# Mehooz/vision4leg

Measured on AMD Instinct MI355X. Metric: PPO env-steps/s (encoder+update, sim excluded), higher is better.
Workload: dtype f16; 1 GPU; ppo_locotransformer thin-goal: LocoTransformer S=93 A=6, E=32 envs x T=512, B=1024, 3 opt epochs; net=loco, envs_per_gpu=32, horizon=512, minibatch=1024, opt_epochs=3, parallelism=dp1, includes_rollout_inference=True, logp_old=recorded at action time (target_pf forward skipped; SURVEY 8d declared saving)

## Files before the change

vision4leg_amd/csrc/bwd.h:

```cpp
#pragma once
#include "infer.h"

namespace v4l {

struct BwdLayer {
  const void *w2t, *w1t, *wot, *wint;
  const float *g1, *g2;
  const float* dy;
  const float *s_qkv, *s_P, *s_xh1, *s_rs1, *s_xh2, *s_rs2;
  const void* s_f;
  void *o_dz2, *o_df, *o_dz1, *o_dqkv;
  float* o_dx;
  float *gp2, *bp2, *gp1, *bp1;
};

struct BwdLayerStack { BwdLayer l[2]; };

struct BwdHead {
  const void *w2t, *w1t, *w0t;
  const float* dout;
  const float *s_h1, *s_h0;
  float *o_dh1, *o_dh0;
};
struct BwdTail {
// ... 632 lines not shown
  LAY_STAMP(8);
  }
  if constexpr (TAIL) {
    __syncthreads();
    {
      f32x4 acc[MT][1];
      zero_acc(acc);
      block_gemm<T, MT, 1, 2>(acc, at, LY::LDX, (const T*)tl.wupt, 64, nt1, lane, ring_up);
      const int n4 = wave * 16 + qr;
#pragma unroll
      for (int mt = 0; mt < MT; ++mt) {
        const int row = mt * 16 + fr;
        const int sm = row / NTOK, t = row - sm * NTOK;
        const bool ok = row < nrows && t > 0;
        const int64_t o = ok ? ((int64_t)(s0 + sm) * 16 + (t - 1)) * TD + n4 : 0;
        const float4 m = tm_c3[mt];
        if (ok)
          st4(tl.o_dc3 + o, m.x > 0.f ? acc[mt][0][0] : 0.f, m.y > 0.f ? acc[mt][0][1] : 0.f, m.z > 0.f ? acc[mt][0][2] : 0.f,
              m.w > 0.f ? acc[mt][0][3] : 0.f);
      }
    }
    float* dt = big;
    T* dh = reinterpret_cast<T*>(big + 16 * LY::LDX);
    GemmRing<T, 4, 8> ring_f2 = gemm_prefetch<T, 4, 8>((const T*)tl.wf2t, 256, nt4, lane);
    __syncthreads();
#pragma unroll
    for (int k = 0; k < 4; ++k) {
      const int idx = tid + k * 256, r = idx >> 6, c = idx & 63;
      dt[r * LY::LDX + c] = r < ns && tm_x0[k] > 0.f ? at[(r * NTOK) * LY::LDX + c] : 0.f;
    }
    __syncthreads();
    f32x4 acc[1][4];
    auto masked = [&](const float4 (&m)[4], T* dst, float* save) {
      const bool ok = fr < ns;
#pragma unroll
      for (int j = 0; j < 4; ++j) {
        const int n4 = nt4[j] * 16 + qr;
        const float d0 = m[j].x > 0.f ? acc[0][j][0] : 0.f, d1 = m[j].y > 0.f ? acc[0][j][1] : 0.f;
        const float d2 = m[j].z > 0.f ? acc[0][j][2] : 0.f, d3 = m[j].w > 0.f ? acc[0][j][3] : 0.f;
        if (dst != nullptr) st4(dst + fr * LY::LDF + n4, d0, d1, d2, d3);
        if (ok) st4(save + (int64_t)(s0 + fr) * 256 + n4, d0, d1, d2, d3);
      }
    };
    zero_acc(acc);
    block_gemm<T, 1, 4, 2>(acc, dt, LY::LDX, (const T*)tl.wpt, 64, nt4, lane, ring_pr);
    masked(tm_e1, dh, tl.o_dhc);
    __syncthreads();
    zero_acc(acc);
    block_gemm<T, 1, 4, 8>(acc, dh, LY::LDF, (const T*)tl.wf2t, 256, nt4, lane, ring_f2);
    masked(tm_e0, (T*)nullptr, tl.o_de0);
  }
  LAY_STAMP(9);
}


struct BwdConv {
  const void* w3d;
  const void* w2d[4];
  const void* image;
  const int* rowidx;
  const float *c1, *c2;
  const float* dc3;
  float *slab1, *slab2, *slab3;
  float *bslab1, *bslab2, *bslab3;
  int n;
  void *t_dc2, *t_dc1;
};
template <typename T> struct BwdConvLds {
  static constexpr bool B16 = sizeof(T) == 2;
  static constexpr int LF = 64 + 4;
  static constexpr int LC1 = 32 + (B16 ? 8 : 0);
  static constexpr int IMGP = B16 ? 1 : 2;
  static constexpr int LT = 64 + (B16 ? 8 : 4);
  static constexpr int LP2 = 64 + (B16 ? 8 : 4);
  static constexpr int LP1 = 256 + (B16 ? 8 : 4);
  static constexpr size_t dc3_b = (size_t)17 * LT * sizeof(T);
  static constexpr size_t c2_b = (size_t)36 * LF * 4;
  static constexpr size_t dc2_b = (size_t)48 * LT * sizeof(T);
  static constexpr size_t dc2T_b = (size_t)64 * LP2 * sizeof(T);
  static constexpr size_t c1_b = ((size_t)225 * LC1 * sizeof(T) + 15) / 16 * 16;
  static constexpr size_t dc1_b = (size_t)32 * LP1 * sizeof(T);
  static constexpr size_t img_b = (size_t)(4 / IMGP) * 4096 * sizeof(T);
  static constexpr size_t w2_b = B16 ? (size_t)4 * 32 * 256 * sizeof(T) : 0;
  static constexpr size_t bytes = dc3_b + c2_b + dc2_b + dc2T_b + c1_b + dc1_b + img_b + w2_b;
  static_assert(bytes <= 160 * 1024, "one block per CU");
};

template <typename T> __device__ __forceinline__ typename Frag<T>::type frag_of(const float (&v)[8]) {
  typename Frag<T>::type f;
  if constexpr (sizeof(T) == 2) {
#pragma unroll
    for (int j = 0; j < 8; ++j) f[j] = (T)v[j];
  } else {
#pragma unroll
    for (int j = 0; j < 8; ++j) f.v[j] = v[j];
  }
  return f;
}
template <typename H>
__device__ __forceinline__ typename Frag<H>::type frag_of_t(const H (&v)[8]) {
  static_assert(sizeof(H) == 2, "16-bit operand type");
  typename Frag<H>::type f;
#pragma unroll
  for (int j = 0; j < 8; ++j) f[j] = v[j];
  return f;
}
__device__ __forceinline__ f32x8 frag_of_t(const float (&v)[8]) { return frag_of<float>(v); }

template <typename T, int MT, int NT, int KS, int KS0 = 0, int PDEPTH = 4, class RowF>
__device__ __forceinline__ void gather_gemm(f32x4 (&acc)[MT][NT], const T* __restrict__ W, int Kp, int nt0, int lane, RowF arow) {
  typedef typename Frag<T>::type frag_t;
  constexpr int PD = NT >= 2 ? 2 : (KS < PDEPTH ? KS : PDEPTH);
  const int fr = lane & 15, fg = (lane >> 4) * 8;
  const T* wrow = W + (int64_t)(nt0 * 16 + fr) * Kp + fg + KS0 * 32;
  frag_t fb[PD][NT];
#pragma unroll
  for (int d = 0; d < PD; ++d)
#pragma unroll
    for (int j = 0; j < NT; ++j) fb[d][j] = *reinterpret_cast<const frag_t*>(wrow + (int64_t)j * 16 * Kp + d * 32);
#pragma unroll
  for (int ks = 0; ks < KS; ++ks) {
    frag_t cur[NT];
#pragma unroll
    for (int j = 0; j < NT; ++j) cur[j] = fb[ks % PD][j];
    if (ks + PD < KS) {
#pragma unroll
      for (int j = 0; j < NT; ++j) fb[ks % PD][j] = *reinterpret_cast<const frag_t*>(wrow + (int64_t)j * 16 * Kp + (ks + PD) * 32);
    }
#pragma unroll
    for (int mt = 0; mt < MT; ++mt) {
      const frag_t fa = *reinterpret_cast<const frag_t*>(arow(mt, (ks + KS0) >> 1) + ((ks + KS0) & 1) * 32 + fg);
#pragma unroll
      for (int j = 0; j < NT; ++j)
        mma_k32(acc[mt][j], cur[j], fa);
    }
  }
}

#ifdef V4L_INFER_TIMING
#define CONV_STAMP(i) do { if (blockIdx.x == 0 && threadIdx.x == 0 && smp == 3 * (int)gridDim.x) g_inf_stamps[16 + (i)] = clock64(); } while (0)
#else
#define CONV_STAMP(i)
#endif
template <typename T, bool A16 = false>
__global__ __launch_bounds__(512) void bwd_conv_kernel(BwdConv a) {
  static_assert(!A16 || sizeof(T) == 2, "A16: activations saved in the bf16 operand type");
  typedef BwdConvLds<T> LY;
  typedef typename Frag<T>::type frag_t;
  constexpr int NTH = 512;
  extern __shared__ __attribute__((aligned(16))) unsigned char smem[];
  T* sdc3 = reinterpret_cast<T*>(smem);
  float* sc2 = reinterpret_cast<float*>(smem + LY::dc3_b);
  T* sdc2t = reinterpret_cast<T*>(smem + LY::dc3_b + LY::c2_b);
  T* sdc2T = reinterpret_cast<T*>(smem + LY::dc3_b + LY::c2_b + LY::dc2_b);
  constexpr size_t o_c1 = LY::dc3_b + LY::c2_b + LY::dc2_b + LY::dc2T_b;
  T* sc1 = reinterpret_cast<T*>(smem + o_c1);
  T* sdc1T = reinterpret_cast<T*>(smem + o_c1 + LY::c1_b);
  T* simg = reinterpret_cast<T*>(smem + o_c1 + LY::c1_b + LY::dc1_b);
  T* sw2 = reinterpret_cast<T*>(smem + o_c1 + LY::c1_b + LY::dc1_b + LY::img_b);
  const int tid = threadIdx.x, lane = tid & 63, wave = tid >> 6;
  const int fr = lane & 15, g = lane >> 4, qr = g * 4;
  const int kt2 = wave * 4;
  const int ch1 = wave >> 1, th1 = wave & 1;
  f32x4 acc2[4][4], acc1[2][2];
#pragma unroll
  for (int t = 0; t < 4; ++t) {
#pragma unroll
    for (int c = 0; c < 4; ++c) acc2[t][c] = f32x4{0.f, 0.f, 0.f, 0.f};
    acc1[t >> 1][t & 1] = f32x4{0.f, 0.f, 0.f, 0.f};
  }
  float b2r[4] = {0.f, 0.f, 0.f, 0.f};
  float b1r[4] = {0.f, 0.f, 0.f, 0.f};
  for (int i = tid; i < 12 * LY::LT; i += NTH) sdc2t[36 * LY::LT + i] = (T)0.f;
  for (int i = tid; i < 64 * LY::LP2; i += NTH) sdc2T[i] = (T)0.f;
  for (int i = tid; i < 32 * LY::LP1; i += NTH) sdc1T[i] = (T)0.f;
  for (int i = tid; i < LY::LT; i += NTH) sdc3[16 * LY::LT + i] = (T)0.f;
  constexpr int CH = 4 / LY::IMGP;

  constexpr int V = 16 / sizeof(T);
  constexpr int N4 = 225 * 8, PT = (N4 + NTH - 1) / NTH;
  constexpr int N8 = 225 * 4, PT8 = (N8 + NTH - 1) / NTH;
  typedef typename Frag<T>::type chunk_t;
  float4 hv0 = float4{0.f, 0.f, 0.f, 0.f}, hv1 = hv0, cv[A16 ? 1 : PT];
  chunk_t h16 = {}, c16[A16 ? PT8 : 1] = {};
  auto load_next = [&](int sm) {
    const float* g3 = a.dc3 + (int64_t)sm * 16 * 64;
    if constexpr (A16) {
      const chunk_t* g2 = reinterpret_cast<const chunk_t*>(reinterpret_cast<const T*>(a.c2) + (int64_t)sm * 36 * 64);
      const chunk_t* g1 = reinterpret_cast<const chunk_t*>(reinterpret_cast<const T*>(a.c1) + (int64_t)sm * 225 * 32);
      h16 = g2[tid < 288 ? tid : 0];
      if (tid >= 256) hv1 = *reinterpret_cast<const float4*>(g3 + (tid - 256) * 4);
#pragma unroll
      for (int k = 0; k < PT8; ++k) {
        const int i8 = tid + k * NTH;
        c16[k] = g1[i8 < N8 ? i8 : 0];
      }
    } else {
      const float* g2 = a.c2 + (int64_t)sm * 36 * 64;
      const float* g1 = a.c1 + (int64_t)sm * 225 * 32;
      hv0 = *reinterpret_cast<const float4*>(g2 + tid * 4);
      if (tid >= 256) hv1 = *reinterpret_cast<const float4*>(g3 + (tid - 256) * 4);
      else if (tid < 64) hv1 = *reinterpret_cast<const float4*>(g2 + (512 + tid) * 4);
#pragma unroll
      for (int k = 0; k < PT; ++k) {
        const int i4 = tid + k * NTH;
        cv[k] = *reinterpret_cast<const float4*>(g1 + (i4 < N4 ? i4 : 0) * 4);
      }
    }
  };
  auto store_next = [&]() {
    if constexpr (A16) {
      if (tid < 288) {
        float* d = sc2 + (tid >> 3) * LY::LF + (tid & 7) * 8;
        *reinterpret_cast<float4*>(d) = float4{(float)h16[0], (float)h16[1], (float)h16[2], (float)h16[3]};
        *reinterpret_cast<float4*>(d + 4) = float4{(float)h16[4], (float)h16[5], (float)h16[6], (float)h16[7]};
      }
      if (tid >= 256) st4(sdc3 + ((tid - 256) >> 4) * LY::LT + (tid & 15) * 4, hv1.x, hv1.y, hv1.z, hv1.w);
#pragma unroll
      for (int k = 0; k < PT8; ++k) {
        const int i8 = tid + k * NTH;
        if (i8 < N8) *reinterpret_cast<chunk_t*>(sc1 + (i8 >> 2) * LY::LC1 + (i8 & 3) * 8) = c16[k];
      }
    } else {
      *reinterpret_cast<float4*>(sc2 + (tid >> 4) * LY::LF + (tid & 15) * 4) = hv0;
      if (tid >= 256) st4(sdc3 + ((tid - 256) >> 4) * LY::LT + (tid & 15) * 4, hv1.x, hv1.y, hv1.z, hv1.w);
      else if (tid < 64) *reinterpret_cast<float4*>(sc2 + (32 + (tid >> 4)) * LY::LF + (tid & 15) * 4) = hv1;
#pragma unroll
      for (int k = 0; k < PT; ++k) {
        const int i4 = tid + k * NTH;
        if (i4 < N4) st4(sc1 + (i4 >> 3) * LY::LC1 + (i4 & 7) * 4, cv[k].x, cv[k].y, cv[k].z, cv[k].w);
      }
    }
  };
  {
    const bool first = (int)blockIdx.x < a.n;
    if (first) load_next(blockIdx.x);
    if constexpr (LY::B16) {
      float4 wv[4096 / NTH];
#pragma unroll
      for (int k = 0; k < 4096 / NTH; ++k) {
        const int c = tid + k * NTH, k8 = c & 31, n = (c >> 5) & 31, cl = c >> 10;
        wv[k] = *reinterpret_cast<const float4*>(reinterpret_cast<const T*>(a.w2d[cl]) + n * 256 + k8 * 8);
      }
#pragma unroll
      for (int k = 0; k < 4096 / NTH; ++k) {
        const int c = tid + k * NTH, k8 = c & 31, n = (c >> 5) & 31, cl = c >> 10;
        const int dst = ((cl * 2 + (n >> 4)) * 8 + (k8 >> 2)) * 64 + (k8 & 3) * 16 + (n & 15);
        *reinterpret_cast<float4*>(sw2 + dst * 8) = wv[k];
      }
    }
    if (first) store_next();
  }
  for (int smp = blockIdx.x; smp < a.n; smp += gridDim.x) {
    __syncthreads();
    CONV_STAMP(0);
    const int64_t slot = a.rowidx != nullptr ? a.rowidx[smp] : smp;
    const T* gimg = reinterpret_cast<const T*>(a.image) + slot * 16384;
    CONV_STAMP(1);
    {
      const int nt = wave & 3;
      const T* W = reinterpret_cast<const T*>(a.w3d);
      int iy[3], ix[3];
      bool okr[3];
#pragma unroll
      for (int m = 0; m < 3; ++m) {
        const int px = m * 16 + fr;
        okr[m] = px < 36;
        iy[m] = px / 6; ix[m] = px - iy[m] * 6;
      }
      f32x4 acc[3][1];
#pragma unroll
      for (int m = 0; m < 3; ++m) acc[m][0] = f32x4{0.f, 0.f, 0.f, 0.f};
      auto arow = [&](int m, int tap) -> const T* {
        const int ta = tap / 3, tb = tap - ta * 3;
        const int oy = iy[m] - ta, ox = ix[m] - tb;
        const bool ok = okr[m] && oy >= 0 && oy < 4 && ox >= 0 && ox < 4;
        return sdc3 + (ok ? oy * 4 + ox : 16) * LY::LT;
      };
      float4* part = reinterpret_cast<float4*>(simg);
      if (wave >= 4) {
        gather_gemm<T, 3, 1, 9, 9, LY::B16 ? 9 : 3>(acc, W, 576, nt, lane, arow);
#pragma unroll
        for (int m = 0; m < 3; ++m) part[(nt * 3 + m) * 64 + lane] = float4{acc[m][0][0], acc[m][0][1], acc[m][0][2], acc[m][0][3]};
      } else {
        gather_gemm<T, 3, 1, 9, 0, LY::B16 ? 9 : 3>(acc, W, 576, nt, lane, arow);
      }
      __syncthreads();
      if (wave < 4) {
#pragma unroll
        for (int m = 0; m < 3; ++m) {
          const int px = m * 16 + fr, c4 = nt * 16 + qr;
          if (px < 36) {
            const float4 hi = part[(nt * 3 + m) * 64 + lane];
            const float4 mk = *reinterpret_cast<const float4*>(sc2 + px * LY::LF + c4);
            const float d0 = mk.x > 0.f ? acc[m][0][0] + hi.x : 0.f, d1 = mk.y > 0.f ? acc[m][0][1] + hi.y : 0.f;
            const float d2 = mk.z > 0.f ? acc[m][0][2] + hi.z : 0.f, d3 = mk.w > 0.f ? acc[m][0][3] + hi.w : 0.f;
            st4(sdc2t + px * LY::LT + c4, d0, d1, d2, d3);
            if (a.t_dc2 != nullptr) st4(reinterpret_cast<T*>(a.t_dc2) + ((int64_t)smp * 36 + px) * 64 + c4, d0, d1, d2, d3);
            T* tp = sdc2T + c4 * LY::LP2 + px;
            tp[0] = (T)d0; tp[LY::LP2] = (T)d1; tp[2 * LY::LP2] = (T)d2; tp[3 * LY::LP2] = (T)d3;
            b2r[0] += d0; b2r[1] += d1; b2r[2] += d2; b2r[3] += d3;
          }
        }
      }
    }
    __syncthreads();
    CONV_STAMP(2);
#pragma unroll
    for (int k = 0; k < CH * 4096 / V / NTH; ++k)
      __builtin_amdgcn_global_load_lds((const V4L_GLOBAL void*)(gimg + (int64_t)(tid + k * NTH) * V),
                                       (__attribute__((address_space(3))) void*)(simg + ((tid & ~63) + k * NTH) * V), 16, 0, 0);
#pragma unroll
    for (int st = 0; st < 2; ++st) {
      frag_t fy[4];
#pragma unroll
      for (int c = 0; c < 4; ++c) fy[c] = *reinterpret_cast<const frag_t*>(sdc2T + (c * 16 + fr) * LY::LP2 + st * 32 + g * 8);
#pragma unroll
      for (int t = 0; t < 4; ++t) {
        const int kt = kt2 + t, tap = kt >> 1, ci = (kt & 1) * 16 + fr;
        const int ky = tap >> 2, kx = tap & 3;
        T w[8];
#pragma unroll
        for (int j = 0; j < 8; ++j) {
          const int pos = st * 32 + g * 8 + j;
          const int pp = pos < 36 ? pos : 0, oy = pp / 6, ox = pp - oy * 6;
          w[j] = sc1[((2 * oy + ky) * 15 + 2 * ox + kx) * LY::LC1 + ci];
        }
        const frag_t fx = frag_of_t(w);
#pragma unroll
        for (int c = 0; c < 4; ++c) mma_k32(acc2[t][c], fx, fy[c]);
      }
    }
    CONV_STAMP(3);
    {
      const int cls = wave >> 1, py = cls >> 1, pxx = cls & 1, nh = wave & 1;
      const int nIy = (15 - py + 1) >> 1, nIx = (15 - pxx + 1) >> 1;
      int ry[4], rx[4];
#pragma unroll
      for (int m = 0; m < 4; ++m) { const int r = m * 16 + fr; ry[m] = r >> 3; rx[m] = r & 7; }
      f32x4 acc[4][1];
#pragma unroll
      for (int m = 0; m < 4; ++m) acc[m][0] = f32x4{0.f, 0.f, 0.f, 0.f};
      auto arow = [&](int m, int tap) -> const T* {
        const int oy = ry[m] - (tap >> 1), ox = rx[m] - (tap & 1);
        const bool ok = ry[m] < nIy && rx[m] < nIx && oy >= 0 && oy < 6 && ox >= 0 && ox < 6;
        return sdc2t + (ok ? oy * 6 + ox : 36) * LY::LT;
      };
      if constexpr (LY::B16) {
        const T* wl = sw2 + (cls * 2 + nh) * 8 * 512 + lane * 8;
#pragma unroll
        for (int ks = 0; ks < 8; ++ks) {
          const frag_t fw = *reinterpret_cast<const frag_t*>(wl + ks * 512);
#pragma unroll
          for (int m = 0; m < 4; ++m)
            mma_k32(acc[m][0], fw, *reinterpret_cast<const frag_t*>(arow(m, ks >> 1) + (ks & 1) * 32 + g * 8));
        }
      } else {
        gather_gemm<T, 4, 1, 8>(acc, reinterpret_cast<const T*>(a.w2d[cls]), 256, nh, lane, arow);
      }
#pragma unroll
      for (int m = 0; m < 4; ++m) {
        if (ry[m] < nIy && rx[m] < nIx) {
          const int p = (py + 2 * ry[m]) * 15 + pxx + 2 * rx[m];
          const int c4 = nh * 16 + qr;
          const float4 mk = ld4(sc1 + p * LY::LC1 + c4);
          const float d0 = mk.x > 0.f ? acc[m][0][0] : 0.f, d1 = mk.y > 0.f ? acc[m][0][1] : 0.f;
          const float d2 = mk.z > 0.f ? acc[m][0][2] : 0.f, d3 = mk.w > 0.f ? acc[m][0][3] : 0.f;
          T* tp = sdc1T + c4 * LY::LP1 + p;
          tp[0] = (T)d0; tp[LY::LP1] = (T)d1; tp[2 * LY::LP1] = (T)d2; tp[3 * LY::LP1] = (T)d3;
          if (a.t_dc1 != nullptr) st4(reinterpret_cast<T*>(a.t_dc1) + ((int64_t)smp * 225 + p) * 32 + c4, d0, d1, d2, d3);
          b1r[0] += d0; b1r[1] += d1; b1r[2] += d2; b1r[3] += d3;
        }
      }
    }
    __syncthreads();
    CONV_STAMP(4);
    CONV_STAMP(5);
    const bool more = smp + (int)gridDim.x < a.n;
    if (more) load_next(smp + gridDim.x);
#pragma unroll 1
    for (int h = 0; h < LY::IMGP; ++h) {
      if (h > 0) {
        __syncthreads();
        for (int i = tid; i < CH * 4096 / V; i += NTH)
          *reinterpret_cast<float4*>(simg + i * V) = *reinterpret_cast<const float4*>(gimg + (int64_t)h * CH * 4096 + i * V);
        __syncthreads();
      }
      if (ch1 >= h * CH && ch1 < (h + 1) * CH) {
        const T* ich = simg + (ch1 - h * CH) * 4096;
#pragma unroll 1
        for (int st = 0; st < 8; ++st) {
          frag_t fy[2];
#pragma unroll
          for (int c = 0; c < 2; ++c) fy[c] = *reinterpret_cast<const frag_t*>(sdc1T + (c * 16 + fr) * LY::LP1 + st * 32 + g * 8);
          int po2[8];
#pragma unroll
          for (int j = 0; j < 8; ++j) {
            const int pos = st * 32 + g * 8 + j;
            const int pp = pos < 225 ? pos : 0, oy = pp / 15, ox = pp - oy * 15;
            po2[j] = (4 * oy) * 64 + 4 * ox;
          }
#pragma unroll
          for (int tt = 0; tt < 2; ++tt) {
            const int ky = (th1 * 2 + tt) * 2 + (fr >> 3), kx = fr & 7;
            T w[8];
#pragma unroll
            for (int j = 0; j < 8; ++j) w[j] = ich[po2[j] + ky * 64 + kx];
            const frag_t fx = frag_of_t(w);
#pragma unroll
            for (int c = 0; c < 2; ++c) mma_k32(acc1[c][tt], fx, fy[c]);
          }
        }
      }
    }
    if (more) store_next();
    CONV_STAMP(6);
  }
  {
    float* o2 = a.slab2 + (int64_t)blockIdx.x * 64 * 512;
#pragma unroll
    for (int t = 0; t < 4; ++t)
#pragma unroll
      for (int c = 0; c < 4; ++c)
        *reinterpret_cast<float4*>(o2 + (c * 16 + fr) * 512 + (kt2 + t) * 16 + qr) =
            float4{acc2[t][c][0], acc2[t][c][1], acc2[t][c][2], acc2[t][c][3]};
    float* o1 = a.slab1 + (int64_t)blockIdx.x * 32 * 256;
#pragma unroll
    for (int c = 0; c < 2; ++c)
#pragma unroll
      for (int tt = 0; tt < 2; ++tt)
        *reinterpret_cast<float4*>(o1 + (c * 16 + fr) * 256 + (ch1 * 4 + th1 * 2 + tt) * 16 + qr) =
            float4{acc1[c][tt][0], acc1[c][tt][1], acc1[c][tt][2], acc1[c][tt][3]};
    __syncthreads();
    float* red2 = reinterpret_cast<float*>(sdc1T);
    float* red1 = red2 + 64 * 16;
    static_assert(LY::dc1_b >= (64 * 16 + 32 * 64) * 4, "bias reduction scratch");
    if (wave < 4) {
#pragma unroll
      for (int i = 0; i < 4; ++i) red2[((wave & 3) * 16 + qr + i) * 16 + fr] = b2r[i];
    }
#pragma unroll
    for (int i = 0; i < 4; ++i) red1[((wave & 1) * 16 + qr + i) * 64 + (wave >> 1) * 16 + fr] = b1r[i];
    __syncthreads();
    if (tid < 64) {
      float t = 0.f;
#pragma unroll
      for (int k = 0; k < 16; ++k) t += red2[tid * 16 + k];
      a.bslab2[(int64_t)blockIdx.x * 64 + tid] = t;
    }
    if (tid < 32) {
      float t = 0.f;
#pragma unroll 8
      for (int k = 0; k < 64; ++k) t += red1[tid * 64 + k];
      a.bslab1[(int64_t)blockIdx.x * 32 + tid] = t;
    }
  }
}

template <typename T, bool A16 = false>
__global__ __launch_bounds__(256) void bwd_conv3_wgrad_kernel(BwdConv a) {
  typedef typename Frag<T>::type frag_t;
  constexpr int LF = 64 + 4;
// ... 104 lines not shown
```

vision4leg_amd/csrc/v4l_hip.hip:

```cpp
#include <math.h>
#include <stdarg.h>

#include <algorithm>
#include <type_traits>

#include <dlfcn.h>

#include "net.h"
#include "infer.h"
#include "bwd.h"
#include "wps.h"
#include "wps_fb.h"
#include "rollout_dense.h"
#include "dense_stack.h"
#include "host_step.h"

namespace v4l {

static thread_local char g_err[1024] = "";
static bool sw_on(const char* name) { return getenv(name) != nullptr; }
template <typename T> struct TypeTag { typedef T type; };
#ifdef V4L_DEV_ONLY
template <class F> static inline int by_compute(int compute, F&& f) {
  typedef std::conditional<V4L_DEV_ONLY == V4L_BF16, __bf16, std::conditional<V4L_DEV_ONLY == V4L_F16, _Float16, float>::type>::type T;
// ... 478 lines not shown
      ep.mask = acts[i - 1].p;
      ep.ldmask = acts[i - 1].ld;
      ep.mask_mode = epi_mask_mode(c.net);
      if ((rc = lin_dgrad<T>(c, Ls[i], y, ep))) return rc;
      y = dense(dbufs[i - 1], acts[i - 1].w, y.M, acts[i - 1].w);
    } else if (din != nullptr) {
      if ((rc = lin_dgrad<T>(c, Ls[0], y, *din))) return rc;
    }
  }
  return 0;
}

static int ln_bwd_launch(Ctx& c, int nblk, const float* dout, float* dz, const float* xhat, const float* rstd, const LNp& ln,
                         int rows) {
  v4l_net* net = c.net;
  float* gpart = c.slab + c.slab_used;
  float* bpart = gpart + (int64_t)nblk * TD;
  c.slab_used += 2 * (int64_t)nblk * TD;
  V4L_REQUIRE(c.slab_used <= net->slab_cap, "internal: weight-grad slab arena overflow");
  V4L_KLAUNCH("ln_bwd", 0, c.s, ln_bwd_kernel, dim3(nblk), dim3(256), 0, c.s, dout, xhat, rstd, net->p[ln.g], rows, dz, gpart,
              bpart);
  V4L_LAUNCH_CHECK();
  for (int k = 0; k < 2; ++k) {
    RedDesc d;
    memset(&d, 0, sizeof(d));
    d.slab = k == 0 ? gpart : bpart;
    d.dW = c.grads + net->params[k == 0 ? ln.g : ln.b].goff;
    d.nsplit = nblk; d.N = 1; d.K = TD; d.Npad = 1; d.Kpad = TD; d.Ktorch = TD;
    net->red.push_back(d);
  }
  return 0;
}

static inline AIm2colNHWC nhwc_loader(const float* p, const Conv& cv, int n) {
  AIm2colNHWC a;
  a.p = p; a.IH = cv.IH; a.IW = cv.IH; a.Cin = cv.Cin; a.OH = cv.OH; a.OW = cv.OH; a.KH = cv.KH; a.KW = cv.KH;
  a.stride = cv.stride; a.M = n * cv.OH * cv.OH; a.K = cv.K;
  return a;
}
template <typename T>
static inline AIm2colCHW<T> chw_loader(const T* img, const Conv& cv, int n, const int* rowidx) {
  AIm2colCHW<T> a;
  a.p = img; a.C = cv.Cin; a.IH = cv.IH; a.IW = cv.IH; a.OH = cv.OH; a.OW = cv.OH; a.stride = cv.stride;
  a.M = n * cv.OH * cv.OH; a.rowidx = rowidx;
  return a;
}

template <typename T>
static int conv_stack_fwd(const Ctx& c, const T* image, const int* rowidx, int n, float* c1, float* c2, float* c3) {
  const v4l_net* N = c.net;
  const Conv* cv = N->conv;
  int rc;
  {
    Epi ep = mk_epi(c1, cv[0].Cout, cv[0].Cout, N->p[cv[0].b], 1);
    auto al = chw_loader<T>(image, cv[0], n, rowidx);
    g_op = "conv1.fwd";
    rc = launch_nt<T>(c.s, al, al.M, (const T*)N->packed + cv[0].pk, cv[0].Np, cv[0].Kp, ep, 2.0 * al.M * cv[0].Cout * cv[0].K);
    if (rc) return rc;
  }
  float* ins[3] = {nullptr, c1, c2};
  float* outs[3] = {c1, c2, c3};
  for (int i = 1; i < 3; ++i) {
    Epi ep = mk_epi(outs[i], cv[i].Cout, cv[i].Cout, N->p[cv[i].b], 1);
    auto al = nhwc_loader(ins[i], cv[i], n);
    g_op = i == 1 ? "conv2.fwd" : "conv3.fwd";
    rc = launch_nt<T>(c.s, al, al.M, (const T*)N->packed + cv[i].pk, cv[i].Np, cv[i].Kp, ep, 2.0 * al.M * cv[i].Cout * cv[i].K);
    if (rc) return rc;
  }
  return 0;
}

static bool conv_bwd_fusable(const v4l_net* N) {
  const Conv* v = N->conv;
  return v[1].Rd == 32 && v[1].Kdp == 256 && v[2].Rd == 64 && v[2].Kdp == 576 && v[0].chw && v[0].Cin == 4 && v[0].IH == 64 && v[0].KH == 8 && v[0].stride == 4 && v[0].Cout == 32 &&
         v[1].Cin == 32 && v[1].KH == 4 && v[1].stride == 2 && v[1].Cout == 64 && v[1].OH == 6 &&
         v[2].Cin == 64 && v[2].KH == 3 && v[2].stride == 1 && v[2].Cout == 64 && v[2].OH == 4 &&
         !sw_on("V4L_NO_FUSED_CONV_BWD");
}
template <typename T>
static int conv_stack_bwd_fused(Ctx& c, const T* image, const int* rowidx, int n, const float* c1, const float* c2,
                                const float* dc3, float* dc2_tap, float* dc1_tap) {
  v4l_net* N = c.net;
  V4L_HIP_CHECK(lds_limit<&bwd_conv_kernel<T>>(BwdConvLds<T>::bytes));
  if constexpr (sizeof(T) == 2) V4L_HIP_CHECK(lds_limit<&bwd_conv_kernel<T, true>>(BwdConvLds<T>::bytes));
  const bool a16 = sizeof(T) == 2 && N->acts16_c1 != nullptr && N->acts16_c1 == c1;
  int nblk = std::min(n, CONV_BWD_MAX_BLOCKS);
  if (const char* e = getenv("V4L_CONV_BWD_BLOCKS")) nblk = std::max(1, std::min(nblk, atoi(e)));
  int nblk3 = std::min(nblk, c.wps_used ? 96 : 160);
  if (const char* e = getenv("V4L_CONV3_WGRAD_BLOCKS")) nblk3 = std::max(1, std::min(nblk, atoi(e)));
  const int Ns[3] = {32, 64, 64}, Ks[3] = {256, 512, 576};
  float* slab[3];
  float* bslab[3];
  for (int i = 0; i < 3; ++i) {
    const int nb = i == 2 ? nblk3 : nblk;
    const int64_t sf = ((int64_t)nb * Ns[i] * Ks[i] + 63) / 64 * 64, bf = ((int64_t)nb * Ns[i] + 63) / 64 * 64;
    slab[i] = c.slab + c.slab_used;
    bslab[i] = slab[i] + sf;
    c.slab_used += sf + bf;
    const Conv& v = N->conv[i];
    RedDesc o;
    memset(&o, 0, sizeof(o));
    o.dW = c.grads + N->params[v.w].goff;
    o.db = c.grads + N->params[v.b].goff;
    o.N = v.Cout; o.K = v.K; o.Ktorch = v.K;
    o.Cin = v.chw ? 0 : v.Cin; o.taps = v.chw ? 0 : v.KH * v.KH;
    o.slab = slab[i]; o.bslab = bslab[i]; o.nsplit = nb; o.Npad = Ns[i]; o.Kpad = Ks[i];
    o.group = 1;
    N->red.push_back(o);
  }
  V4L_REQUIRE(c.slab_used <= N->slab_cap, "internal: weight-grad slab arena overflow");
  BwdConv a;
  memset(&a, 0, sizeof(a));
  a.w3d = (const T*)N->packed + N->conv[2].pkd[0];
  for (int cls = 0; cls < 4; ++cls) a.w2d[cls] = (const T*)N->packed + N->conv[1].pkd[cls];
  a.image = image; a.rowidx = rowidx; a.c1 = c1; a.c2 = c2; a.dc3 = dc3;
  if (c.taps) { a.t_dc2 = dc2_tap; a.t_dc1 = dc1_tap; }
  a.slab1 = slab[0]; a.slab2 = slab[1]; a.slab3 = slab[2];
  a.bslab1 = bslab[0]; a.bslab2 = bslab[1]; a.bslab3 = bslab[2];
  a.n = n;
  g_op = "conv.bwd";
  const double fl = 2.0 * n * (16.0 * 64 * 576 + 2.0 * 36 * 64 * 512 + 225.0 * 32 * 256);
  if constexpr (sizeof(T) == 2) {
    if (a16) V4L_KLAUNCH("fused_conv_bwd", fl, c.s, (bwd_conv_kernel<T, true>), dim3(nblk), dim3(512), BwdConvLds<T>::bytes, c.s, a);
  }
  if (!a16) V4L_KLAUNCH("fused_conv_bwd", fl, c.s, bwd_conv_kernel<T>, dim3(nblk), dim3(512), BwdConvLds<T>::bytes, c.s, a);
  V4L_LAUNCH_CHECK();
  if (c.defer_conv3) {
    c.conv3_args = a; c.conv3_blocks = nblk3; c.conv3_n = n; c.conv3_pending = true; c.conv3_a16 = a16;
    return 0;
  }
  g_op = "conv3.wgrad";
  if constexpr (sizeof(T) == 2) {
    if (a16) V4L_KLAUNCH("fused_conv3_wgrad", 2.0 * n * 16 * 64 * 576, c.tn, (bwd_conv3_wgrad_kernel<T, true>), dim3(nblk3), dim3(256), 0, c.tn, a);
  }
  if (!a16) V4L_KLAUNCH("fused_conv3_wgrad", 2.0 * n * 16 * 64 * 576, c.tn, bwd_conv3_wgrad_kernel<T>, dim3(nblk3), dim3(256), 0, c.tn, a);
  V4L_LAUNCH_CHECK();
  return 0;
}
template <typename T>
static int conv3_wgrad_deferred(Ctx& c, hipStream_t s) {
  if (!c.conv3_pending) return 0;
  c.conv3_pending = false;
  g_op = "conv3.wgrad";
  if constexpr (sizeof(T) == 2) {
    if (c.conv3_a16)
      V4L_KLAUNCH("fused_conv3_wgrad", 2.0 * c.conv3_n * 16 * 64 * 576, s, (bwd_conv3_wgrad_kernel<T, true>), dim3(c.conv3_blocks),
                  dim3(256), 0, s, c.conv3_args);
  }
  if (!c.conv3_a16)
    V4L_KLAUNCH("fused_conv3_wgrad", 2.0 * c.conv3_n * 16 * 64 * 576, s, bwd_conv3_wgrad_kernel<T>, dim3(c.conv3_blocks), dim3(256), 0, s,
                c.conv3_args);
  V4L_LAUNCH_CHECK();
  return 0;
}

template <typename T>
static int conv_stack_bwd(Ctx& c, const T* image, const int* rowidx, int n, const float* c1, const float* c2,
                          float* dc3, float* dc2, float* dc1) {
  if (conv_bwd_fusable(c.net)) return conv_stack_bwd_fused<T>(c, image, rowidx, n, c1, c2, dc3, dc2, dc1);
  const v4l_net* N = c.net;
  const Conv* cv = N->conv;
  const float* acts[3] = {nullptr, c1, c2};
  float* dys[3] = {dc1, dc2, dc3};
  for (int i = 2; i >= 0; --i) {
    const Conv& v = cv[i];
    const int M = n * v.OH * v.OH;
    ADense y = dense(dys[i], v.Cout, M, v.Cout);
    RedDesc o;
    memset(&o, 0, sizeof(o));
    o.dW = c.grads + N->params[v.w].goff;
    o.db = c.grads + N->params[v.b].goff;
    o.N = v.Cout; o.K = v.K; o.Ktorch = v.K;
    int rc;
    if (i > 0 && (rc = par_begin(c))) return rc;
    if (v.chw) {
      o.Cin = 0; o.taps = 0;
      auto x = chw_loader<T>(image, v, n, rowidx);
      g_op = "conv1.wgrad";
      rc = launch_tn<T>(c, y, x, M, v.Cout, v.K, o, 2.0 * M * v.Cout * v.K);
    } else {
      o.Cin = v.Cin; o.taps = v.KH * v.KH;
      auto x = nhwc_loader(acts[i], v, n);
      g_op = i == 1 ? "conv2.wgrad" : "conv3.wgrad";
      rc = launch_tn<T>(c, y, x, M, v.Cout, v.K, o, 2.0 * M * v.Cout * v.K);
    }
    if (rc) return rc;
    if (i == 0) break;
    const int st = v.stride, TH = v.KH / st;
    DgradClasses<T> dc;
    memset(&dc, 0, sizeof(dc));
    dc.Kp = v.Kdp;
    int maxM = 0;
    for (int cls = 0; cls < v.ncls; ++cls) {
      const int py = cls / st, px = cls % st;
      ADgradNHWC& a = dc.a[cls];
      a.p = dys[i]; a.OH = v.OH; a.OW = v.OH; a.Cout = v.Cout; a.TH = TH; a.TW = TH;
      a.nIy = (v.IH - py + st - 1) / st; a.nIx = (v.IH - px + st - 1) / st;
      a.M = n * a.nIy * a.nIx; a.K = v.Kd;
      Epi ep = mk_epi(dys[i - 1], v.Cin, v.Cin);
      ep.M = a.M;
      ep.rowmap = ROWMAP_DGRAD;
      ep.py = py; ep.px = px; ep.s = st; ep.nIy = a.nIy; ep.nIx = a.nIx; ep.IH = v.IH; ep.IW = v.IH;
      ep.mask = acts[i]; ep.ldmask = v.Cin;
      dc.ep[cls] = ep;
      dc.B[cls] = (const T*)N->packed + v.pkd[cls];
      maxM = std::max(maxM, a.M);
    }
    g_op = i == 1 ? "conv2.dgrad" : "conv3.dgrad";
// ... 3098 lines not shown
```

Before: 416,300 env-steps/s.

## Batch conv3 data-grad over four-sample chunks with register-held weights in fused conv bwd

Adds a CHUNK variant of the fused conv backward kernel, on by default for 16-bit types. Every fourth iteration it computes the conv3 input-gradient for up to four samples at once, keeping the conv3 weight fragments in registers and splitting the K dimension across two wave halves with an LDS partial-sum exchange. Results for the later samples are stashed in LDS and replayed on the following iterations, so the weights are not reloaded for every sample. In exchange the LDS layout changes (stash overlays the head buffers, chunk operands reuse the image buffer), barriers are added and control flow becomes uneven across iterations.

```diff
diff --git a/vision4leg_amd/csrc/bwd.h b/vision4leg_amd/csrc/bwd.h
--- a/vision4leg_amd/csrc/bwd.h
+++ b/vision4leg_amd/csrc/bwd.h
@@ -738,8 +738,13 @@
   static constexpr size_t dc1_b = (size_t)32 * LP1 * sizeof(T);
   static constexpr size_t img_b = (size_t)(4 / IMGP) * 4096 * sizeof(T);
   static constexpr size_t w2_b = B16 ? (size_t)4 * 32 * 256 * sizeof(T) : 0;
-  static constexpr size_t bytes = dc3_b + c2_b + dc2_b + dc2T_b + c1_b + dc1_b + img_b + w2_b;
-  static_assert(bytes <= 160 * 1024, "one block per CU");
+  static constexpr size_t stash_b = B16 ? (size_t)3 * 36 * 64 * sizeof(T) : 0;
+  static constexpr size_t head_b = dc3_b + c2_b > stash_b ? dc3_b + c2_b : stash_b;
+  static constexpr size_t cdc3_b = (size_t)65 * LT * sizeof(T);
+  static constexpr int PARTN = 4 * (64 + 64 + 16);
+  static_assert(!B16 || (cdc3_b % 16 == 0 && cdc3_b + 2 * PARTN * 16 <= img_b), "chunk operands fit the image buffer");
+  static constexpr size_t bytes = head_b + dc2_b + dc2T_b + c1_b + dc1_b + img_b + w2_b;
+  static_assert(bytes <= 160 * 1024, "one block per CU (with the stash)");
 };
 
 template <typename T> __device__ __forceinline__ typename Frag<T>::type frag_of(const float (&v)[8]) {
@@ -795,21 +800,38 @@
 
 #ifdef V4L_INFER_TIMING
 #define CONV_STAMP(i) do { if (blockIdx.x == 0 && threadIdx.x == 0 && smp == 3 * (int)gridDim.x) g_inf_stamps[16 + (i)] = clock64(); } while (0)
+#define CONV_HEAD_STAMP(i) do { if (blockIdx.x == 0 && threadIdx.x == 0 && smp == 0) g_inf_stamps[24 + (i)] = clock64(); } while (0)
 #else
 #define CONV_STAMP(i)
+#define CONV_HEAD_STAMP(i)
 #endif
-template <typename T, bool A16 = false>
+template <typename T, int KS0, class RowF>
+__device__ __forceinline__ void conv3_held_gemm(f32x4 (&acc)[3][1], const typename Frag<T>::type (&fw)[9], int lane, RowF arow) {
+  typedef typename Frag<T>::type frag_t;
+  const int fg = (lane >> 4) * 8;
+#pragma unroll
+  for (int ks = 0; ks < 9; ++ks) {
+#pragma unroll
+    for (int mt = 0; mt < 3; ++mt) {
+      const frag_t fa = *reinterpret_cast<const frag_t*>(arow(mt, (ks + KS0) >> 1) + ((ks + KS0) & 1) * 32 + fg);
+      mma_k32(acc[mt][0], fw[ks], fa);
+    }
+  }
+}
+template <typename T, bool A16 = false, bool CHUNK = false>
 __global__ __launch_bounds__(512) void bwd_conv_kernel(BwdConv a) {
   static_assert(!A16 || sizeof(T) == 2, "A16: activations saved in the bf16 operand type");
+  static_assert(!CHUNK || sizeof(T) == 2, "CHUNK: the stash takes the place of the fp32 mask rows");
   typedef BwdConvLds<T> LY;
   typedef typename Frag<T>::type frag_t;
   constexpr int NTH = 512;
   extern __shared__ __attribute__((aligned(16))) unsigned char smem[];
   T* sdc3 = reinterpret_cast<T*>(smem);
   float* sc2 = reinterpret_cast<float*>(smem + LY::dc3_b);
-  T* sdc2t = reinterpret_cast<T*>(smem + LY::dc3_b + LY::c2_b);
-  T* sdc2T = reinterpret_cast<T*>(smem + LY::dc3_b + LY::c2_b + LY::dc2_b);
-  constexpr size_t o_c1 = LY::dc3_b + LY::c2_b + LY::dc2_b + LY::dc2T_b;
+  T* stash = reinterpret_cast<T*>(smem);
+  T* sdc2t = reinterpret_cast<T*>(smem + LY::head_b);
+  T* sdc2T = reinterpret_cast<T*>(smem + LY::head_b + LY::dc2_b);
+  constexpr size_t o_c1 = LY::head_b + LY::dc2_b + LY::dc2T_b;
   T* sc1 = reinterpret_cast<T*>(smem + o_c1);
   T* sdc1T = reinterpret_cast<T*>(smem + o_c1 + LY::c1_b);
   T* simg = reinterpret_cast<T*>(smem + o_c1 + LY::c1_b + LY::dc1_b);
@@ -830,8 +852,10 @@
   for (int i = tid; i < 12 * LY::LT; i += NTH) sdc2t[36 * LY::LT + i] = (T)0.f;
   for (int i = tid; i < 64 * LY::LP2; i += NTH) sdc2T[i] = (T)0.f;
   for (int i = tid; i < 32 * LY::LP1; i += NTH) sdc1T[i] = (T)0.f;
-  for (int i = tid; i < LY::LT; i += NTH) sdc3[16 * LY::LT + i] = (T)0.f;
+  if constexpr (!CHUNK)
+    for (int i = tid; i < LY::LT; i += NTH) sdc3[16 * LY::LT + i] = (T)0.f;
   constexpr int CH = 4 / LY::IMGP;
+  const int G = gridDim.x;
 
   constexpr int V = 16 / sizeof(T);
   constexpr int N4 = 225 * 8, PT = (N4 + NTH - 1) / NTH;
@@ -844,8 +868,10 @@
     if constexpr (A16) {
       const chunk_t* g2 = reinterpret_cast<const chunk_t*>(reinterpret_cast<const T*>(a.c2) + (int64_t)sm * 36 * 64);
       const chunk_t* g1 = reinterpret_cast<const chunk_t*>(reinterpret_cast<const T*>(a.c1) + (int64_t)sm * 225 * 32);
-      h16 = g2[tid < 288 ? tid : 0];
-      if (tid >= 256) hv1 = *reinterpret_cast<const float4*>(g3 + (tid - 256) * 4);
+      if constexpr (!CHUNK) {
+        h16 = g2[tid < 288 ? tid : 0];
+        if (tid >= 256) hv1 = *reinterpret_cast<const float4*>(g3 + (tid - 256) * 4);
+      }
 #pragma unroll
       for (int k = 0; k < PT8; ++k) {
         const int i8 = tid + k * NTH;
@@ -854,9 +880,11 @@
     } else {
       const float* g2 = a.c2 + (int64_t)sm * 36 * 64;
       const float* g1 = a.c1 + (int64_t)sm * 225 * 32;
-      hv0 = *reinterpret_cast<const float4*>(g2 + tid * 4);
-      if (tid >= 256) hv1 = *reinterpret_cast<const float4*>(g3 + (tid - 256) * 4);
-      else if (tid < 64) hv1 = *reinterpret_cast<const float4*>(g2 + (512 + tid) * 4);
+      if constexpr (!CHUNK) {
+        hv0 = *reinterpret_cast<const float4*>(g2 + tid * 4);
+        if (tid >= 256) hv1 = *reinterpret_cast<const float4*>(g3 + (tid - 256) * 4);
+        else if (tid < 64) hv1 = *reinterpret_cast<const float4*>(g2 + (512 + tid) * 4);
+      }
 #pragma unroll
       for (int k = 0; k < PT; ++k) {
         const int i4 = tid + k * NTH;
@@ -866,31 +894,50 @@
   };
   auto store_next = [&]() {
     if constexpr (A16) {
-      if (tid < 288) {
-        float* d = sc2 + (tid >> 3) * LY::LF + (tid & 7) * 8;
-        *reinterpret_cast<float4*>(d) = float4{(float)h16[0], (float)h16[1], (float)h16[2], (float)h16[3]};
-        *reinterpret_cast<float4*>(d + 4) = float4{(float)h16[4], (float)h16[5], (float)h16[6], (float)h16[7]};
-      }
-      if (tid >= 256) st4(sdc3 + ((tid - 256) >> 4) * LY::LT + (tid & 15) * 4, hv1.x, hv1.y, hv1.z, hv1.w);
+      if constexpr (!CHUNK) {
+        if (tid < 288) {
+          float* d = sc2 + (tid >> 3) * LY::LF + (tid & 7) * 8;
+          *reinterpret_cast<float4*>(d) = float4{(float)h16[0], (float)h16[1], (float)h16[2], (float)h16[3]};
+          *reinterpret_cast<float4*>(d + 4) = float4{(float)h16[4], (float)h16[5], (float)h16[6], (float)h16[7]};
+        }
+        if (tid >= 256) st4(sdc3 + ((tid - 256) >> 4) * LY::LT + (tid & 15) * 4, hv1.x, hv1.y, hv1.z, hv1.w);
+      }
 #pragma unroll
       for (int k = 0; k < PT8; ++k) {
         const int i8 = tid + k * NTH;
         if (i8 < N8) *reinterpret_cast<chunk_t*>(sc1 + (i8 >> 2) * LY::LC1 + (i8 & 3) * 8) = c16[k];
       }
     } else {
-      *reinterpret_cast<float4*>(sc2 + (tid >> 4) * LY::LF + (tid & 15) * 4) = hv0;
-      if (tid >= 256) st4(sdc3 + ((tid - 256) >> 4) * LY::LT + (tid & 15) * 4, hv1.x, hv1.y, hv1.z, hv1.w);
-      else if (tid < 64) *reinterpret_cast<float4*>(sc2 + (32 + (tid >> 4)) * LY::LF + (tid & 15) * 4) = hv1;
+      if constexpr (!CHUNK) {
+        *reinterpret_cast<float4*>(sc2 + (tid >> 4) * LY::LF + (tid & 15) * 4) = hv0;
+        if (tid >= 256) st4(sdc3 + ((tid - 256) >> 4) * LY::LT + (tid & 15) * 4, hv1.x, hv1.y, hv1.z, hv1.w);
+        else if (tid < 64) *reinterpret_cast<float4*>(sc2 + (32 + (tid >> 4)) * LY::LF + (tid & 15) * 4) = hv1;
+      }
 #pragma unroll
       for (int k = 0; k < PT; ++k) {
         const int i4 = tid + k * NTH;
         if (i4 < N4) st4(sc1 + (i4 >> 3) * LY::LC1 + (i4 & 7) * 4, cv[k].x, cv[k].y, cv[k].z, cv[k].w);
       }
     }
+  };
+  T* cdc3 = simg;
+  float4* part = reinterpret_cast<float4*>(reinterpret_cast<unsigned char*>(simg) + LY::cdc3_b);
+  auto load_chunk = [&](int sm0) {
+    const int s0 = sm0 + (tid >> 8) * G, s1 = s0 + 2 * G;
+    hv0 = hv1 = float4{0.f, 0.f, 0.f, 0.f};
+    if (s0 < a.n) hv0 = *reinterpret_cast<const float4*>(a.dc3 + (int64_t)s0 * 16 * 64 + (tid & 255) * 4);
+    if (s1 < a.n) hv1 = *reinterpret_cast<const float4*>(a.dc3 + (int64_t)s1 * 16 * 64 + (tid & 255) * 4);
+  };
+  auto file_chunk = [&]() {
+    T* d = cdc3 + (tid >> 4) * LY::LT + (tid & 15) * 4;
+    st4(d, hv0.x, hv0.y, hv0.z, hv0.w);
+    st4(d + 32 * LY::LT, hv1.x, hv1.y, hv1.z, hv1.w);
+    if (tid < LY::LT / 4) st4(cdc3 + 64 * LY::LT + tid * 4, 0.f, 0.f, 0.f, 0.f);
   };
   {
     const bool first = (int)blockIdx.x < a.n;
     if (first) load_next(blockIdx.x);
+    if constexpr (CHUNK) load_chunk(blockIdx.x);
     if constexpr (LY::B16) {
       float4 wv[4096 / NTH];
 #pragma unroll
@@ -907,13 +954,105 @@
     }
     if (first) store_next();
   }
-  for (int smp = blockIdx.x; smp < a.n; smp += gridDim.x) {
+  int ci = 0;
+  for (int smp = blockIdx.x; smp < a.n; smp += G, ci = (ci + 1) & 3) {
     __syncthreads();
     CONV_STAMP(0);
     const int64_t slot = a.rowidx != nullptr ? a.rowidx[smp] : smp;
     const T* gimg = reinterpret_cast<const T*>(a.image) + slot * 16384;
     CONV_STAMP(1);
-    {
+    if constexpr (CHUNK) {
+      if (ci == 0) {
+        CONV_HEAD_STAMP(0);
+        file_chunk();
+        __syncthreads();
+        CONV_HEAD_STAMP(1);
+        const int cn = min(4, (a.n - 1 - smp) / G + 1);
+        const int nt = wave & 3, c4 = nt * 16 + qr;
+        const bool hiw = wave >= 4;
+        frag_t fw[9];
+        {
+          const T* wrow = reinterpret_cast<const T*>(a.w3d) + (nt * 16 + fr) * 576 + g * 8 + (hiw ? 9 * 32 : 0);
+#pragma unroll
+          for (int k = 0; k < 9; ++k) fw[k] = *reinterpret_cast<const frag_t*>(wrow + k * 32);
+        }
+        int iy[3], ix[3];
+        bool okr[3];
+#pragma unroll
+        for (int m = 0; m < 3; ++m) {
+          const int px = m * 16 + fr;
+          okr[m] = px < 36;
+          iy[m] = px / 6; ix[m] = px - iy[m] * 6;
+        }
+        int pslot[3];
+        pslot[0] = nt * 144 + lane; pslot[1] = pslot[0] + 64; pslot[2] = nt * 144 + 128 + g * 4 + (fr & 3);
+#pragma unroll 1
+        for (int i = 0; i < cn; ++i) {
+          const int sm = smp + i * G;
+          typedef typename std::conditional<A16, typename HVec<T, 4>::type, float4>::type mask_t;
+          mask_t mk[3] = {};
+          if (!hiw) {
+#pragma unroll
+            for (int m = 0; m < 3; ++m) {
+              const int64_t o = ((int64_t)sm * 36 + (okr[m] ? m * 16 + fr : 0)) * 64 + c4;
+              if constexpr (A16) mk[m] = *reinterpret_cast<const mask_t*>(reinterpret_cast<const T*>(a.c2) + o);
+              else mk[m] = *reinterpret_cast<const mask_t*>(a.c2 + o);
+            }
+          }
+          f32x4 acc[3][1];
+#pragma unroll
+          for (int m = 0; m < 3; ++m) acc[m][0] = f32x4{0.f, 0.f, 0.f, 0.f};
+          const T* rows = cdc3 + i * 16 * LY::LT;
+          auto arow = [&](int m, int tap) -> const T* {
+            const int ta = tap / 3, tb = tap - ta * 3;
+            const int oy = iy[m] - ta, ox = ix[m] - tb;
+            const bool ok = okr[m] && oy >= 0 && oy < 4 && ox >= 0 && ox < 4;
+            return ok ? rows + (oy * 4 + ox) * LY::LT : cdc3 + 64 * LY::LT;
+          };
+          float4* pb = part + (i & 1) * LY::PARTN;
+          if (hiw) {
+            conv3_held_gemm<T, 9>(acc, fw, lane, arow);
+#pragma unroll
+            for (int m = 0; m < 3; ++m)
+              if (m < 2 || fr < 4) pb[pslot[m]] = float4{acc[m][0][0], acc[m][0][1], acc[m][0][2], acc[m][0][3]};
+          } else {
+            conv3_held_gemm<T, 0>(acc, fw, lane, arow);
+          }
+          __syncthreads();
+          if (!hiw) {
+#pragma unroll
+            for (int m = 0; m < 3; ++m) {
+              const int px = m * 16 + fr;
+              if (px < 36) {
+                const float4 hi = pb[pslot[m]];
+                float4 mf;
+                if constexpr (A16) mf = float4{(float)mk[m][0], (float)mk[m][1], (float)mk[m][2], (float)mk[m][3]};
+                else mf = mk[m];
+                const float d0 = mf.x > 0.f ? acc[m][0][0] + hi.x : 0.f, d1 = mf.y > 0.f ? acc[m][0][1] + hi.y : 0.f;
+                const float d2 = mf.z > 0.f ? acc[m][0][2] + hi.z : 0.f, d3 = mf.w > 0.f ? acc[m][0][3] + hi.w : 0.f;
+                if (i == 0) {
+                  st4(sdc2t + px * LY::LT + c4, d0, d1, d2, d3);
+                  T* tp = sdc2T + c4 * LY::LP2 + px;
+                  tp[0] = (T)d0; tp[LY::LP2] = (T)d1; tp[2 * LY::LP2] = (T)d2; tp[3 * LY::LP2] = (T)d3;
+                } else {
+                  st4(stash + (i - 1) * 36 * 64 + px * 64 + c4, d0, d1, d2, d3);
+                }
+                if (a.t_dc2 != nullptr) st4(reinterpret_cast<T*>(a.t_dc2) + ((int64_t)sm * 36 + px) * 64 + c4, d0, d1, d2, d3);
+                b2r[0] += d0; b2r[1] += d1; b2r[2] += d2; b2r[3] += d3;
+              }
+            }
+          }
+        }
+        CONV_HEAD_STAMP(2);
+      } else if (tid < 288) {
+        const int px = tid >> 3, c8 = (tid & 7) * 8;
+        const frag_t v = *reinterpret_cast<const frag_t*>(stash + (ci - 1) * 36 * 64 + tid * 8);
+        *reinterpret_cast<frag_t*>(sdc2t + px * LY::LT + c8) = v;
+        T* tp = sdc2T + c8 * LY::LP2 + px;
+#pragma unroll
+        for (int j = 0; j < 8; ++j) tp[j * LY::LP2] = v[j];
+      }
+    } else {
       const int nt = wave & 3;
       const T* W = reinterpret_cast<const T*>(a.w3d);
       int iy[3], ix[3];
@@ -1034,6 +1173,9 @@
     CONV_STAMP(5);
     const bool more = smp + (int)gridDim.x < a.n;
     if (more) load_next(smp + gridDim.x);
+    if constexpr (CHUNK) {
+      if (more && ci == 3) load_chunk(smp + G);
+    }
 #pragma unroll 1
     for (int h = 0; h < LY::IMGP; ++h) {
       if (h > 0) {
diff --git a/vision4leg_amd/csrc/v4l_hip.hip b/vision4leg_amd/csrc/v4l_hip.hip
--- a/vision4leg_amd/csrc/v4l_hip.hip
+++ b/vision4leg_amd/csrc/v4l_hip.hip
@@ -584,7 +584,12 @@
                                 const float* dc3, float* dc2_tap, float* dc1_tap) {
   v4l_net* N = c.net;
   V4L_HIP_CHECK(lds_limit<&bwd_conv_kernel<T>>(BwdConvLds<T>::bytes));
-  if constexpr (sizeof(T) == 2) V4L_HIP_CHECK(lds_limit<&bwd_conv_kernel<T, true>>(BwdConvLds<T>::bytes));
+  if constexpr (sizeof(T) == 2) {
+    V4L_HIP_CHECK(lds_limit<&bwd_conv_kernel<T, true>>(BwdConvLds<T>::bytes));
+    V4L_HIP_CHECK(lds_limit<&bwd_conv_kernel<T, false, true>>(BwdConvLds<T>::bytes));
+    V4L_HIP_CHECK(lds_limit<&bwd_conv_kernel<T, true, true>>(BwdConvLds<T>::bytes));
+  }
+  const bool chunked = sizeof(T) == 2 && !sw_on("V4L_CONV3_PER_SAMPLE");
   const bool a16 = sizeof(T) == 2 && N->acts16_c1 != nullptr && N->acts16_c1 == c1;
   int nblk = std::min(n, CONV_BWD_MAX_BLOCKS);
   if (const char* e = getenv("V4L_CONV_BWD_BLOCKS")) nblk = std::max(1, std::min(nblk, atoi(e)));
@@ -623,9 +628,11 @@
   g_op = "conv.bwd";
   const double fl = 2.0 * n * (16.0 * 64 * 576 + 2.0 * 36 * 64 * 512 + 225.0 * 32 * 256);
   if constexpr (sizeof(T) == 2) {
-    if (a16) V4L_KLAUNCH("fused_conv_bwd", fl, c.s, (bwd_conv_kernel<T, true>), dim3(nblk), dim3(512), BwdConvLds<T>::bytes, c.s, a);
-  }
-  if (!a16) V4L_KLAUNCH("fused_conv_bwd", fl, c.s, bwd_conv_kernel<T>, dim3(nblk), dim3(512), BwdConvLds<T>::bytes, c.s, a);
+    if (chunked && a16) V4L_KLAUNCH("fused_conv_bwd", fl, c.s, (bwd_conv_kernel<T, true, true>), dim3(nblk), dim3(512), BwdConvLds<T>::bytes, c.s, a);
+    if (chunked && !a16) V4L_KLAUNCH("fused_conv_bwd", fl, c.s, (bwd_conv_kernel<T, false, true>), dim3(nblk), dim3(512), BwdConvLds<T>::bytes, c.s, a);
+    if (!chunked && a16) V4L_KLAUNCH("fused_conv_bwd", fl, c.s, (bwd_conv_kernel<T, true>), dim3(nblk), dim3(512), BwdConvLds<T>::bytes, c.s, a);
+  }
+  if (!chunked && !a16) V4L_KLAUNCH("fused_conv_bwd", fl, c.s, bwd_conv_kernel<T>, dim3(nblk), dim3(512), BwdConvLds<T>::bytes, c.s, a);
   V4L_LAUNCH_CHECK();
   if (c.defer_conv3) {
     c.conv3_args = a; c.conv3_blocks = nblk3; c.conv3_n = n; c.conv3_pending = true; c.conv3_a16 = a16;
```

Measured after the change: 401,100 env-steps/s. 0.963x the previous value.
